# OpenVVC/OpenVVC

Measured on AMD Instinct MI355X. Metric: decoded frames/sec, full rcn back-end decode step (H2D of the recorded picture + MC incl. BDOF/DMVR/affine-PROF/GPM/CIIP + LMCS + inverse transform + ordered intra pass + deblocking + SAO + ALF/CC-ALF + D2H of refined MVs + wait + per-picture digest + publication to the device DPB), 4K 10-bit RA rec, higher is better.
Workload: dtype u16 samples / int16 coefficients / int32 accumulate

## Files before the change

### openvvc_amd/csrc/kernels_alf.hip

```cpp
#include "ovvc_common.hip.h"

#ifndef OV_WPE_ALF
#define OV_WPE_ALF 0
#endif
#if OV_WPE_ALF > 0
#define OV_OCC_ALF __attribute__((amdgpu_waves_per_eu(OV_WPE_ALF)))
#else
#define OV_OCC_ALF
#endif

namespace {

#define TL 32
#define LH 3
#define LW (TL + 2 * LH)
#define LPAD 4
#define LWS 40
#define CH 2
#define CW (TL + 2 * CH)

struct AlfRect { int x0, y0, x1, y1; };
__device__ __forceinline__ AlfRect alf_clamp_rect(int border, int x0, int y0, int s, int w, int h)
{
    AlfRect r = { 0, 0, w - 1, h - 1 };
    if (border & OVHIP_BORDER_LEFT) r.x0 = x0;
    if (border & OVHIP_BORDER_UPPER) r.y0 = y0;
    if (border & OVHIP_BORDER_RIGHT) r.x1 = min(r.x1, x0 + s - 1);
    if (border & OVHIP_BORDER_BOTTOM) r.y1 = min(r.y1, y0 + s - 1);
    return r;
}

__device__ __forceinline__ int alf_clipd(int clip, int ref, int a, int b)
// ... 28 lines not shown
    const int act = min((int)(((sum_h + sum_v) * scale) >> (OV_BD + 4)), 15);
    int c = act == 0 ? 0 : act == 1 ? 1 : act <= 6 ? 2 : act <= 14 ? 3 : 4;
    uint32_t max_hv, min_hv, max_db, min_db, max_dir, min_dir;
    int dir_hv, dir_db, main_dir, sec_dir;
    if (sum_v > sum_h) { max_hv = sum_v; min_hv = sum_h; dir_hv = 1; } else { max_hv = sum_h; min_hv = sum_v; dir_hv = 3; }
    if (sum_d > sum_b) { max_db = sum_d; min_db = sum_b; dir_db = 0; } else { max_db = sum_b; min_db = sum_d; dir_db = 2; }
    if (max_db * min_hv > max_hv * min_db) { max_dir = max_db; min_dir = min_db; main_dir = dir_db; sec_dir = dir_hv; }
    else { max_dir = max_hv; min_dir = min_hv; main_dir = dir_hv; sec_dir = dir_db; }
    if (max_dir * 2 > 9 * min_dir) c += (((main_dir & 1) << 1) + 2) * 5;
    else if (max_dir > 2 * min_dir) c += (((main_dir & 1) << 1) + 1) * 5;
    cls = c;
    const int k = (main_dir << 1) + (sec_dir >> 1);
    tr = (0xDE84 >> (2 * k)) & 3;
}

__device__ __forceinline__ void alf_luma_tile(const ovhip_pic &dst, const ovhip_pic &src, const ovhip_alf_pic &alf, int nb_ctu_w,
                                              int tile0, uint16_t *s_t, uint8_t *s_cls, uint4 *s_sum, int row0, int row1)
{

    const int W = src.w, H = src.h;
    const int tid = threadIdx.x;
    const int ctu = 1 << alf.log2_ctu_s;
    const int ntx = (W + TL - 1) / TL, ntiles = ntx * ((H + TL - 1) / TL);
    for (int tile = tile0; tile < ntiles; tile = ntiles) {
    const int tx0 = (tile % ntx) * TL, ty0 = (tile / ntx) * TL;
    const ovhip_alf_ctu c = alf.ctus[(ty0 >> alf.log2_ctu_s) * nb_ctu_w + (tx0 >> alf.log2_ctu_s)];
    const bool on = c.flags & 4;

    const int b = tid >> 2, r = tid & 3;
    const int bx = (b & 7) * 4, by = (b >> 3) * 4;
    const int ox = tx0 + bx, oy = ty0 + by + r;

    if (!on) {
        if (oy < H && oy >= row0 && oy < row1) {
#pragma unroll
            for (int i = 0; i < 4; ++i) if (ox + i < W) dst.y[oy * dst.stride_y + ox + i] = src.y[oy * src.stride_y + ox + i];
        }
        continue;
    }

    const AlfRect rc = alf_clamp_rect(c.border, tx0 & ~(ctu - 1), ty0 & ~(ctu - 1), ctu, W, H);
    if (tx0 >= rc.x0 + LPAD && tx0 + TL + LPAD <= rc.x1 + 1 && ty0 >= rc.y0 + LH && ty0 + TL + LH <= rc.y1 + 1 && !(src.stride_y & 7)) {
        if (tid < LW * 5) {
            const int yy = tid / 5, q = tid - yy * 5;
            *reinterpret_cast<uint4 *>(s_t + yy * LWS + 8 * q) =
                *reinterpret_cast<const uint4 *>(src.y + (ty0 + yy - LH) * src.stride_y + tx0 - LPAD + 8 * q);
        }
    } else {
        for (int i = tid; i < LW * LWS; i += 256) {
            const int yy = i / LWS, xx = i - yy * LWS;
            const int sy = ov_clip3(ty0 + yy - LH, rc.y0, rc.y1), sx = ov_clip3(tx0 + xx - LPAD, rc.x0, rc.x1);
            s_t[i] = src.y[sy * src.stride_y + sx];
        }
    }
    __syncthreads();

    const int ctu_y0 = ty0 & ~(ctu - 1);
    const bool truncated = ctu_y0 + ctu > H;
    const int vbl = truncated ? H : ctu - 4;
    const int last_local = (ctu_y0 + (truncated ? H - ctu_y0 : ctu) - 1) & (ctu - 1);
    const bool req_vb = (last_local < vbl && last_local >= vbl - 4) || (last_local >= vbl && last_local <= vbl + 3);
    const int vb = ctu_y0 + vbl;

#define T(x, y) ((int)s_t[((y) + LH) * LWS + (x) + LPAD])
    {
        const int cb = tid >> 2, k = tid & 3;
        const int cbx = (cb & 7) * 4, cby = (cb >> 3) * 4;
        const int rr = cby - 2 + 2 * k;
        int above = rr - 1, below = rr + 2;
        if (ty0 + rr + 2 == vb) below = rr + 1;
        if (ty0 + rr == vb)     above = rr;
        uint32_t sv = 0, sh = 0, sd = 0, sb = 0;
        {
            uint32_t ra[6], r0[6], r1[6], rb[6];
            const uint16_t *base = s_t + LH * LWS + cbx;
            auto row3 = [&](int y, uint32_t d6[6]) {
                const uint2 *q2 = reinterpret_cast<const uint2 *>(base + y * LWS);
                const uint2 a = q2[0], b_ = q2[1], c_ = q2[2];
                d6[0] = a.x; d6[1] = a.y; d6[2] = b_.x; d6[3] = b_.y; d6[4] = c_.x; d6[5] = c_.y;
            };
            row3(above, ra); row3(rr, r0); row3(rr + 1, r1); row3(below, rb);
            typedef unsigned short alf_u2 __attribute__((ext_vector_type(2)));
#pragma unroll
            for (int q = 0; q < 4; ++q) {
                const int c0 = 2 * q - 2, c1 = c0 + 1;
                const alf_u2 ctr = __builtin_bit_cast(alf_u2, ALF_PK66(r0, c0, r1, c1));
                const uint32_t y2 = __builtin_bit_cast(uint32_t, ctr + ctr);
#define LAP(acc, A, ca, B, cb, C, cc_, D, cd)                                                                      \
                acc = __builtin_amdgcn_sad_u16(y2, __builtin_bit_cast(uint32_t, __builtin_bit_cast(alf_u2, ALF_PK66(A, ca, B, cb)) + \
                                                                               __builtin_bit_cast(alf_u2, ALF_PK66(C, cc_, D, cd))), acc)
                LAP(sv, ra, c0, r0, c1, r1, c0, rb, c1);
                LAP(sh, r0, c0 + 1, r1, c1 + 1, r0, c0 - 1, r1, c1 - 1);
                LAP(sd, ra, c0 - 1, r0, c1 - 1, r1, c0 + 1, rb, c1 + 1);
                LAP(sb, r1, c0 - 1, rb, c1 - 1, ra, c0 + 1, r0, c1 + 1);
#undef LAP
            }
        }
        const int py = ty0 + cby;
        bool use = true, is_vb = false;
        if (py == vb - 4) { is_vb = true; use = k < 3; }
        if (py == vb)     { is_vb = true; use = k > 0; }
        if (!use) sv = sh = sd = sb = 0;
        (void)is_vb;
        s_sum[tid] = make_uint4(sv, sh, sd, sb);
    }
    __syncthreads();
    if (tid < 64) {
        const uint4 p0 = s_sum[4 * tid], p1 = s_sum[4 * tid + 1], p2 = s_sum[4 * tid + 2], p3 = s_sum[4 * tid + 3];
        const int py = ty0 + (tid >> 3) * 4;
        int cls, tr;
        filter_idx(p0.y + p1.y + p2.y + p3.y, p0.x + p1.x + p2.x + p3.x, p0.z + p1.z + p2.z + p3.z, p0.w + p1.w + p2.w + p3.w,
                   py == vb - 4 || py == vb, cls, tr);
        s_cls[tid] = (uint8_t)(cls | (tr << 5));
    }
    __syncthreads();

    if (oy >= H || oy < row0 || oy >= row1) continue;
    const int ct = s_cls[b];
    const int cls = ct & 31, tr = ct >> 5;
    const int16_t *f = alf.luma_coeff + c.luma_set * OVHIP_ALF_LUMA_SET_SIZE + tr * 25 * 13 + cls * 13;
    const int16_t *cl = alf.luma_clip + c.luma_set * OVHIP_ALF_LUMA_SET_SIZE + tr * 25 * 13 + cls * 13;
    typedef uint32_t alf_u32a2 __attribute__((aligned(2)));
    uint32_t fw[6], cw6[6];
#pragma unroll
    for (int j = 0; j < 6; ++j) { fw[j] = *reinterpret_cast<const alf_u32a2 *>(f + 2 * j); cw6[j] = *reinterpret_cast<const alf_u32a2 *>(cl + 2 * j); }

    int d = 3;
    bool near = false;
    if (req_vb) {
        if (oy < vb && oy >= vb - 4) d = vb - 1 - oy;
        else if (oy >= vb && oy <= vb + 3) d = oy - vb;
        near = (oy == vb - 1) || (oy == vb);
    }
    const int o1 = min(d, 1), o2 = min(d, 2), o3 = min(d, 3);
    const int ly = by + r;
    uint32_t r0[6], p1[6], m1[6], p2[6], m2[6], p3[2], m3[2];
    {
        const uint16_t *base = s_t + LH * LWS + bx;
        auto row3 = [&](int y, uint32_t d6[6]) {
            const uint2 *q = reinterpret_cast<const uint2 *>(base + y * LWS);
            const uint2 a = q[0], b_ = q[1], c_ = q[2];
            d6[0] = a.x; d6[1] = a.y; d6[2] = b_.x; d6[3] = b_.y; d6[4] = c_.x; d6[5] = c_.y;
        };
        auto row1 = [&](int y, uint32_t d2[2]) {
            const uint2 a = reinterpret_cast<const uint2 *>(base + y * LWS)[1];
            d2[0] = a.x; d2[1] = a.y;
        };
        row3(ly, r0); row3(ly + o1, p1); row3(ly - o1, m1); row3(ly + o2, p2); row3(ly - o2, m2);
        row1(ly + o3, p3); row1(ly - o3, m3);
    }
#define S6(d6, c) ((((c) + 4) & 1) ? (int)((d6)[((c) + 4) >> 1] >> 16) : (int)((d6)[((c) + 4) >> 1] & 0xffff))
#define S2(d2, c) (((c) & 1) ? (int)((d2)[(c) >> 1] >> 16) : (int)((d2)[(c) >> 1] & 0xffff))
    alf_s2 cm2 = __builtin_bit_cast(alf_s2, cw6[0]);
    int fsum = 0;
#pragma unroll
    for (int j = 1; j < 6; ++j) cm2 = __builtin_elementwise_min(cm2, __builtin_bit_cast(alf_s2, cw6[j]));
#pragma unroll
    for (int j = 0; j < 6; ++j) fsum = __builtin_amdgcn_sdot2(__builtin_bit_cast(alf_s2, fw[j]), (alf_s2)(1), fsum, false);
    const int cmin = min((int)cm2.x, (int)cm2.y);
    const bool linear = __all(cmin > OV_PIX_MAX);
    uint32_t f2[12], c2[12], nc2[12];
#pragma unroll
    for (int j = 0; j < 6; ++j) {
        f2[2 * j] = __builtin_amdgcn_perm(fw[j], fw[j], 0x01000100u); f2[2 * j + 1] = __builtin_amdgcn_perm(fw[j], fw[j], 0x03020302u);
    }
    if (!linear) {
#pragma unroll
        for (int j = 0; j < 6; ++j) {
            c2[2 * j] = __builtin_amdgcn_perm(cw6[j], cw6[j], 0x01000100u); c2[2 * j + 1] = __builtin_amdgcn_perm(cw6[j], cw6[j], 0x03020302u);
        }
#pragma unroll
        for (int i = 0; i < 12; ++i) nc2[i] = __builtin_bit_cast(uint32_t, (alf_s2)(0) - __builtin_bit_cast(alf_s2, c2[i]));
    }
    int outv[4];
#pragma unroll
    for (int i = 0; i < 4; ++i) {
        const int cur = S6(r0, i);
        const uint32_t n[12] = {
            ALF_PK22(p3, i, m3, i),
            ALF_PK66(p2, i + 1, m2, i - 1), ALF_PK66(p2, i, m2, i), ALF_PK66(p2, i - 1, m2, i + 1),
            ALF_PK66(p1, i + 2, m1, i - 2), ALF_PK66(p1, i + 1, m1, i - 1), ALF_PK66(p1, i, m1, i),
            ALF_PK66(p1, i - 1, m1, i + 1), ALF_PK66(p1, i - 2, m1, i + 2),
            ALF_PK66(r0, i + 3, r0, i - 3), ALF_PK66(r0, i + 2, r0, i - 2), ALF_PK66(r0, i + 1, r0, i - 1) };
        int sum;
        if (linear) {
            sum = -2 * cur * fsum;
#pragma unroll
            for (int k = 0; k < 12; ++k) sum = alf_tap_lin(n[k], f2[k], sum);
        } else {
            const uint32_t cur2 = ALF_PK66(r0, i, r0, i);
            sum = 0;
#pragma unroll
            for (int k = 0; k < 12; ++k) sum = alf_tap(n[k], cur2, c2[k], nc2[k], f2[k], sum);
        }
        sum = near ? (sum + 512) >> 10 : (sum + 64) >> 7;
        outv[i] = ov_clip_bd(sum + cur);
    }
#undef S6
#undef S2
    {
        uint16_t *o = dst.y + oy * dst.stride_y + ox;
        if (ox + 3 < W && !(dst.stride_y & 3)) {
            uint2 v; v.x = (uint32_t)outv[0] | ((uint32_t)outv[1] << 16); v.y = (uint32_t)outv[2] | ((uint32_t)outv[3] << 16);
            *reinterpret_cast<uint2 *>(o) = v;
        } else {
#pragma unroll
            for (int i = 0; i < 4; ++i) if (ox + i < W) o[i] = (uint16_t)outv[i];
        }
    }
    }
#undef T
}

__device__ __forceinline__ void alf_chroma_tile(const ovhip_pic &dst, const ovhip_pic &src, const ovhip_alf_pic &alf, int nb_ctu_w,
                                                int tile0, int comp, uint16_t *s_t, int row0, int row1)
{
    const int W = src.w, H = src.h, Wc = W >> 1, Hc = H >> 1;
    const int tid = threadIdx.x;
    const int ctu = 1 << alf.log2_ctu_s, ctuc = ctu >> 1;
    const int ntx = (Wc + TL - 1) / TL, ntiles = ntx * ((Hc + TL - 1) / TL);
    for (int tile = tile0; tile < ntiles; tile = ntiles) {
    const int tx0 = (tile % ntx) * TL, ty0 = (tile / ntx) * TL;
    const ovhip_alf_ctu c = alf.ctus[((ty0 * 2) >> alf.log2_ctu_s) * nb_ctu_w + ((tx0 * 2) >> alf.log2_ctu_s)];
    const bool on = c.flags & (comp == 1 ? 2 : 1);
    const int cc_idx = comp == 1 ? c.cc_cb_idx : c.cc_cr_idx;
    const uint16_t *sp = comp == 1 ? src.cb : src.cr;
// ... 141 lines not shown
#undef S6
#undef S2
    uint16_t *o = dp + oy * dst.stride_c + tx0 + lx0;
    if (tx0 + lx0 + 3 < Wc && !(dst.stride_c & 3)) {
        uint2 v; v.x = (uint32_t)outv[0] | ((uint32_t)outv[1] << 16); v.y = (uint32_t)outv[2] | ((uint32_t)outv[3] << 16);
        *reinterpret_cast<uint2 *>(o) = v;
    } else {
#pragma unroll
        for (int i = 0; i < 4; ++i) if (tx0 + lx0 + i < Wc) o[i] = (uint16_t)outv[i];
    }
    }
}

__global__ __launch_bounds__(256) OV_OCC_ALF void k_alf(ovhip_pic dst, ovhip_pic src, ovhip_alf_pic alf, int nb_ctu_w, int nl, int nc, int t0_l, int t0_c, int row0, int row1)
{
    __shared__ __attribute__((aligned(16))) uint16_t s_t[(LW > CW ? LW : CW) * LWS];
    __shared__ uint8_t s_cls[64];
    __shared__ __attribute__((aligned(16))) uint4 s_sum[256];
    const int b = blockIdx.x;
    if (b < nl) alf_luma_tile(dst, src, alf, nb_ctu_w, t0_l + (int)ov_xcd_slot_at(b, 0, nl), s_t, s_cls, s_sum, row0, row1);
    else {
        const int comp = 1 + (b - nl) / nc;
        alf_chroma_tile(dst, src, alf, nb_ctu_w, t0_c + (int)ov_xcd_slot_at(b, nl + (comp - 1) * nc, nc), comp, s_t, row0, row1);
    }
}

}

extern "C" int ovhip_alf_launch_rows(ovhip_ctx *ctx, const ovhip_pic *dst, const ovhip_pic *src, const ovhip_alf_pic *alf, int32_t row0, int32_t row1)
{
    if (!ctx || !dst || !src || !alf) return OVHIP_EINVAL;
    OV_DEVICE(ctx);
    if (dst->w != src->w || dst->h != src->h || dst->y == src->y || alf->log2_ctu_s < 6 || alf->log2_ctu_s > 7 ||
        !alf->ctus || !alf->luma_coeff || !alf->luma_clip || !alf->chroma_coeff || !alf->chroma_clip || !alf->cc_coeff)
        return ov_fail(ctx, OVHIP_EINVAL, "ovhip_alf_launch: bad pictures / parameter tables", hipSuccess);
    if (row0 < 0 || row1 > src->h || row0 > row1 || (row0 & 7) || ((row1 & 7) && row1 != src->h))
        return ov_fail(ctx, OVHIP_EINVAL, "ovhip_alf_launch_rows: row window", hipSuccess);
    if (row0 == row1) return OVHIP_OK;
    const int nb_ctu_w = (src->w + (1 << alf->log2_ctu_s) - 1) >> alf->log2_ctu_s;
    const int ntx_l = (src->w + TL - 1) / TL, ntx_c = (src->w / 2 + TL - 1) / TL;
    const int ty0_l = row0 / TL, ty1_l = (row1 + TL - 1) / TL, ty0_c = (row0 / 2) / TL, ty1_c = (row1 / 2 + TL - 1) / TL;
    const int nl = ntx_l * (ty1_l - ty0_l), nc = ntx_c * (ty1_c - ty0_c);
    hipLaunchKernelGGL(k_alf, dim3(nl + 2 * nc), dim3(256), 0, ctx->stream, *dst, *src, *alf, nb_ctu_w, nl, nc, ty0_l * ntx_l, ty0_c * ntx_c, row0, row1);
    OV_LAUNCH_CHECK(ctx, "k_alf");
    return OVHIP_OK;
}

extern "C" int ovhip_alf_launch(ovhip_ctx *ctx, const ovhip_pic *dst, const ovhip_pic *src, const ovhip_alf_pic *alf)
{
    if (!src) return OVHIP_EINVAL;
    return ovhip_alf_launch_rows(ctx, dst, src, alf, 0, src->h);
}
```

### openvvc_amd/csrc/kernels_sao.hip

```cpp
#include "ovvc_common.hip.h"
#include <stdlib.h>

namespace {

#define SAO_TW 64
#define SAO_TH 32

struct Vec8 { int v[8]; };

__device__ __forceinline__ void load8(const uint16_t *p, bool vec, int n, int v[8])
{
    if (vec) {
        const uint4 q = *reinterpret_cast<const uint4 *>(p);
        v[0] = q.x & 0xffff; v[1] = q.x >> 16; v[2] = q.y & 0xffff; v[3] = q.y >> 16;
        v[4] = q.z & 0xffff; v[5] = q.z >> 16; v[6] = q.w & 0xffff; v[7] = q.w >> 16;
    } else {
#pragma unroll
        for (int i = 0; i < 8; ++i) v[i] = i < n ? p[i] : 0;
    }
}

__global__ __launch_bounds__(256) void k_sao(ovhip_pic dst, ovhip_pic src, const ovhip_sao_ctu *__restrict__ prm,
                                              int log2_ctu, int nb_ctu_w, int tiles_y, int tiles_c, int ty0_y, int ty0_c, int row0, int row1)
{
    const int tx = threadIdx.x & 7, ty = threadIdx.x >> 3;
    for (int t = blockIdx.x; t < tiles_y + 2 * tiles_c; t = tiles_y + 2 * tiles_c) {
        const int c = t < tiles_y ? 0 : (t < tiles_y + tiles_c ? 1 : 2);
        const int tt = (int)ov_xcd_slot_at(t, c == 0 ? 0 : (c == 1 ? tiles_y : tiles_y + tiles_c), c == 0 ? tiles_y : tiles_c);
        const int sh = c ? 1 : 0;
        const int w = src.w >> sh, h = src.h >> sh, l2 = log2_ctu - sh;
        const int ntx = (w + SAO_TW - 1) / SAO_TW;
        const int x0 = (tt % ntx) * SAO_TW + tx * 8, y = (tt / ntx + (c ? ty0_c : ty0_y)) * SAO_TH + ty;
        if (x0 >= w || y >= h || y < (row0 >> sh) || y >= (row1 >> sh)) continue;
        int ss, ds;
        const uint16_t *s = ov_plane(src, c, ss) + y * ss;
        uint16_t *d = ov_plane(dst, c, ds) + y * ds;
        const ovhip_sao_ctu *p = &prm[(y >> l2) * nb_ctu_w + (x0 >> l2)];
        const int type = p->type[c];
        const int n = min(8, w - x0);
        const bool vec = n == 8 && !((ss | ds) & 7) && !(((uintptr_t)s | (uintptr_t)d) & 15);
        int v[8], o[8];
        load8(s + x0, vec, n, v);
#pragma unroll
        for (int i = 0; i < 8; ++i) o[i] = v[i];
        if (type == OVHIP_SAO_BAND) {
            const int bp = p->band_position[c];
            const int o0 = p->offset_val[c][0], o1 = p->offset_val[c][1], o2 = p->offset_val[c][2], o3 = p->offset_val[c][3];
#pragma unroll
            for (int i = 0; i < 8; ++i) {
                const int k = ((v[i] >> (OV_BD - 5)) - bp) & 31;
                const int off = k == 0 ? o0 : k == 1 ? o1 : k == 2 ? o2 : k == 3 ? o3 : 0;
                o[i] = ov_clip_bd(v[i] + off);
            }
        } else if (type == OVHIP_SAO_EDGE) {
            const int eo = p->eo_class[c];
            const int dxa = eo == 1 ? 0 : (eo == 3 ? 1 : -1), dya = eo == 0 ? 0 : -1;
            const int bd = p->border, cs = 1 << l2;
            const int cy0 = y & ~(cs - 1), cx0 = x0 & ~(cs - 1);
            const int cx1 = min(cx0 + cs, w) - 1;
            const bool rowskip = eo != 0 && (y == 0 || y == h - 1 || (src.h <= (1 << log2_ctu) && y == (6 >> sh) - 1) ||
                                             ((bd & OVHIP_BORDER_UPPER) && y == cy0) || ((bd & OVHIP_BORDER_BOTTOM) && y == min(cy0 + cs, h) - 1) ||
                                             ((bd & OVHIP_BORDER_ONE_ROW) && y == cy0 + (6 >> sh) - 1));
            const int skip_l = (bd & OVHIP_BORDER_LEFT) ? cx0 : -1, skip_r = (bd & OVHIP_BORDER_RIGHT) ? cx1 : -1;
            if (!rowskip) {
                const int of0 = p->offset_val[c][0], of1 = p->offset_val[c][1], of2 = p->offset_val[c][2],
                          of3 = p->offset_val[c][3], of4 = p->offset_val[c][4];
                int ra[10], rb[10];
                const uint16_t *sa = s + dya * ss, *sb = s - dya * ss;
                load8(sa + x0, vec, n, ra + 1);
                load8(sb + x0, vec, n, rb + 1);
                ra[0] = x0 > 0 ? sa[x0 - 1] : 0; rb[0] = x0 > 0 ? sb[x0 - 1] : 0;
                ra[9] = x0 + 8 < w ? sa[x0 + 8] : 0; rb[9] = x0 + 8 < w ? sb[x0 + 8] : 0;
#pragma unroll
                for (int i = 0; i < 8; ++i) {
                    const int x = x0 + i;
                    if (i < n && !(eo != 1 && (x == 0 || x == w - 1 || x == skip_l || x == skip_r))) {
                        const int a = ra[1 + i + dxa], b = rb[1 + i - dxa];
                        const int idx = 2 + (v[i] > a) - (v[i] < a) + (v[i] > b) - (v[i] < b);
                        const int off = idx == 0 ? of0 : idx == 1 ? of1 : idx == 2 ? of2 : idx == 3 ? of3 : of4;
                        o[i] = ov_clip_bd(v[i] + off);
                    }
                }
            }
        }
        if (vec) {
            uint4 q;
            q.x = o[0] | (o[1] << 16); q.y = o[2] | (o[3] << 16); q.z = o[4] | (o[5] << 16); q.w = o[6] | (o[7] << 16);
            *reinterpret_cast<uint4 *>(d + x0) = q;
        } else {
#pragma unroll
            for (int i = 0; i < 8; ++i) if (i < n) d[x0 + i] = (uint16_t)o[i];
        }
    }
}

}

extern "C" int ovhip_sao_launch_rows(ovhip_ctx *ctx, const ovhip_pic *dst, const ovhip_pic *src,
                                     const ovhip_sao_ctu *d_params, int32_t log2_ctu_s, int32_t row0, int32_t row1)
{
    if (!ctx || !dst || !src || !d_params) return OVHIP_EINVAL;
    OV_DEVICE(ctx);
    if (dst->w != src->w || dst->h != src->h || dst->y == src->y || log2_ctu_s < 5 || log2_ctu_s > 7)
        return ov_fail(ctx, OVHIP_EINVAL, "ovhip_sao_launch: bad pictures / CTU size", hipSuccess);
    if (row0 < 0 || row1 > src->h || row0 > row1 || (row0 & 7) || ((row1 & 7) && row1 != src->h))
        return ov_fail(ctx, OVHIP_EINVAL, "ovhip_sao_launch_rows: row window", hipSuccess);
    if (row0 == row1) return OVHIP_OK;
    const int nb_ctu_w = (src->w + (1 << log2_ctu_s) - 1) >> log2_ctu_s;
// ... 18 lines not shown
```

Measured before the change: 3631.

## Enlarge ALF luma tiles to 4x4 per thread and register-block SAO rows

```diff
diff --git a/openvvc_amd/csrc/kernels_alf.hip b/openvvc_amd/csrc/kernels_alf.hip
--- a/openvvc_amd/csrc/kernels_alf.hip
+++ b/openvvc_amd/csrc/kernels_alf.hip
@@ -12,10 +12,12 @@
 namespace {
 
 #define TL 32
+#define TLL 64
 #define LH 3
-#define LW (TL + 2 * LH)
 #define LPAD 4
 #define LWS 40
+#define LLS 72
+#define LLH (TLL + 2 * LH)
 #define CH 2
 #define CW (TL + 2 * CH)
 
@@ -74,46 +76,105 @@
     tr = (0xDE84 >> (2 * k)) & 3;
 }
 
+__device__ __forceinline__ void alf_lap_pair(const uint32_t ra[6], const uint32_t r0[6], const uint32_t r1[6], const uint32_t rb[6],
+                                             uint32_t &sv, uint32_t &sh, uint32_t &sd, uint32_t &sb)
+{
+    typedef unsigned short alf_u2 __attribute__((ext_vector_type(2)));
+#pragma unroll
+    for (int q = 0; q < 4; ++q) {
+        const int c0 = 2 * q - 2, c1 = c0 + 1;
+        const alf_u2 ctr = __builtin_bit_cast(alf_u2, ALF_PK66(r0, c0, r1, c1));
+        const uint32_t y2 = __builtin_bit_cast(uint32_t, ctr + ctr);
+#define LAP(acc, A, ca, B, cb, C, cc_, D, cd)                                                                      \
+        acc = __builtin_amdgcn_sad_u16(y2, __builtin_bit_cast(uint32_t, __builtin_bit_cast(alf_u2, ALF_PK66(A, ca, B, cb)) + \
+                                                                       __builtin_bit_cast(alf_u2, ALF_PK66(C, cc_, D, cd))), acc)
+        LAP(sv, ra, c0, r0, c1, r1, c0, rb, c1);
+        LAP(sh, r0, c0 + 1, r1, c1 + 1, r0, c0 - 1, r1, c1 - 1);
+        LAP(sd, ra, c0 - 1, r0, c1 - 1, r1, c0 + 1, rb, c1 + 1);
+        LAP(sb, r1, c0 - 1, rb, c1 - 1, ra, c0 + 1, r0, c1 + 1);
+#undef LAP
+    }
+}
+
+struct AlfLumaSet { uint32_t f2[12], c2[12], nc2[12]; int fsum; bool linear; };
+
+__device__ __forceinline__ uint2 alf_luma_row(const uint32_t r0[6], const uint32_t p1[6], const uint32_t m1[6], const uint32_t p2[6],
+                                              const uint32_t m2[6], const uint32_t p3[6], const uint32_t m3[6], bool near, const AlfLumaSet &fs)
+{
+#define S6(d6, c) ((((c) + 4) & 1) ? (int)((d6)[((c) + 4) >> 1] >> 16) : (int)((d6)[((c) + 4) >> 1] & 0xffff))
+    int outv[4];
+#pragma unroll
+    for (int i = 0; i < 4; ++i) {
+        const int cur = S6(r0, i);
+        const uint32_t n[12] = {
+            ALF_PK66(p3, i, m3, i),
+            ALF_PK66(p2, i + 1, m2, i - 1), ALF_PK66(p2, i, m2, i), ALF_PK66(p2, i - 1, m2, i + 1),
+            ALF_PK66(p1, i + 2, m1, i - 2), ALF_PK66(p1, i + 1, m1, i - 1), ALF_PK66(p1, i, m1, i),
+            ALF_PK66(p1, i - 1, m1, i + 1), ALF_PK66(p1, i - 2, m1, i + 2),
+            ALF_PK66(r0, i + 3, r0, i - 3), ALF_PK66(r0, i + 2, r0, i - 2), ALF_PK66(r0, i + 1, r0, i - 1) };
+        int sum;
+        if (fs.linear) {
+            sum = -2 * cur * fs.fsum;
+#pragma unroll
+            for (int k = 0; k < 12; ++k) sum = alf_tap_lin(n[k], fs.f2[k], sum);
+        } else {
+            const uint32_t cur2 = ALF_PK66(r0, i, r0, i);
+            sum = 0;
+#pragma unroll
+            for (int k = 0; k < 12; ++k) sum = alf_tap(n[k], cur2, fs.c2[k], fs.nc2[k], fs.f2[k], sum);
+        }
+        sum = near ? (sum + 512) >> 10 : (sum + 64) >> 7;
+        outv[i] = ov_clip_bd(sum + cur);
+    }
+#undef S6
+    uint2 v; v.x = (uint32_t)outv[0] | ((uint32_t)outv[1] << 16); v.y = (uint32_t)outv[2] | ((uint32_t)outv[3] << 16);
+    return v;
+}
+
 __device__ __forceinline__ void alf_luma_tile(const ovhip_pic &dst, const ovhip_pic &src, const ovhip_alf_pic &alf, int nb_ctu_w,
-                                              int tile0, uint16_t *s_t, uint8_t *s_cls, uint4 *s_sum, int row0, int row1)
+                                              int tile0, uint16_t *s_t, int row0, int row1)
 {
 
     const int W = src.w, H = src.h;
     const int tid = threadIdx.x;
     const int ctu = 1 << alf.log2_ctu_s;
-    const int ntx = (W + TL - 1) / TL, ntiles = ntx * ((H + TL - 1) / TL);
+    const int ntx = (W + TLL - 1) / TLL, ntiles = ntx * ((H + TLL - 1) / TLL);
     for (int tile = tile0; tile < ntiles; tile = ntiles) {
-    const int tx0 = (tile % ntx) * TL, ty0 = (tile / ntx) * TL;
+    const int tx0 = (tile % ntx) * TLL, ty0 = (tile / ntx) * TLL;
     const ovhip_alf_ctu c = alf.ctus[(ty0 >> alf.log2_ctu_s) * nb_ctu_w + (tx0 >> alf.log2_ctu_s)];
     const bool on = c.flags & 4;
 
-    const int b = tid >> 2, r = tid & 3;
-    const int bx = (b & 7) * 4, by = (b >> 3) * 4;
-    const int ox = tx0 + bx, oy = ty0 + by + r;
+    const int bx = (tid & 15) * 4, by = (tid >> 4) * 4;
+    const int ox = tx0 + bx, py = ty0 + by;
+    const bool mine = py < H && py >= row0 && py < row1 && ox < W;
 
     if (!on) {
-        if (oy < H && oy >= row0 && oy < row1) {
-#pragma unroll
-            for (int i = 0; i < 4; ++i) if (ox + i < W) dst.y[oy * dst.stride_y + ox + i] = src.y[oy * src.stride_y + ox + i];
+        if (mine) {
+#pragma unroll
+            for (int r = 0; r < 4; ++r)
+#pragma unroll
+                for (int i = 0; i < 4; ++i)
+                    if (py + r < H && ox + i < W) dst.y[(py + r) * dst.stride_y + ox + i] = src.y[(py + r) * src.stride_y + ox + i];
         }
         continue;
     }
 
     const AlfRect rc = alf_clamp_rect(c.border, tx0 & ~(ctu - 1), ty0 & ~(ctu - 1), ctu, W, H);
-    if (tx0 >= rc.x0 + LPAD && tx0 + TL + LPAD <= rc.x1 + 1 && ty0 >= rc.y0 + LH && ty0 + TL + LH <= rc.y1 + 1 && !(src.stride_y & 7)) {
-        if (tid < LW * 5) {
-            const int yy = tid / 5, q = tid - yy * 5;
-            *reinterpret_cast<uint4 *>(s_t + yy * LWS + 8 * q) =
+    if (tx0 >= rc.x0 + LPAD && tx0 + TLL + LPAD <= rc.x1 + 1 && ty0 >= rc.y0 + LH && ty0 + TLL + LH <= rc.y1 + 1 && !(src.stride_y & 7)) {
+        for (int i = tid; i < LLH * 9; i += 256) {
+            const int yy = i / 9, q = i - yy * 9;
+            *reinterpret_cast<uint4 *>(s_t + yy * LLS + 8 * q) =
                 *reinterpret_cast<const uint4 *>(src.y + (ty0 + yy - LH) * src.stride_y + tx0 - LPAD + 8 * q);
         }
     } else {
-        for (int i = tid; i < LW * LWS; i += 256) {
-            const int yy = i / LWS, xx = i - yy * LWS;
+        for (int i = tid; i < LLH * LLS; i += 256) {
+            const int yy = i / LLS, xx = i - yy * LLS;
             const int sy = ov_clip3(ty0 + yy - LH, rc.y0, rc.y1), sx = ov_clip3(tx0 + xx - LPAD, rc.x0, rc.x1);
             s_t[i] = src.y[sy * src.stride_y + sx];
         }
     }
     __syncthreads();
+    if (!mine) continue;
 
     const int ctu_y0 = ty0 & ~(ctu - 1);
     const bool truncated = ctu_y0 + ctu > H;
@@ -121,155 +182,100 @@
     const int last_local = (ctu_y0 + (truncated ? H - ctu_y0 : ctu) - 1) & (ctu - 1);
     const bool req_vb = (last_local < vbl && last_local >= vbl - 4) || (last_local >= vbl && last_local <= vbl + 3);
     const int vb = ctu_y0 + vbl;
-
-#define T(x, y) ((int)s_t[((y) + LH) * LWS + (x) + LPAD])
-    {
-        const int cb = tid >> 2, k = tid & 3;
-        const int cbx = (cb & 7) * 4, cby = (cb >> 3) * 4;
-        const int rr = cby - 2 + 2 * k;
-        int above = rr - 1, below = rr + 2;
-        if (ty0 + rr + 2 == vb) below = rr + 1;
-        if (ty0 + rr == vb)     above = rr;
-        uint32_t sv = 0, sh = 0, sd = 0, sb = 0;
-        {
+    const bool is_vb = py == vb - 4 || py == vb;
+    const bool at_vb = py + 3 >= vb - 4 && py <= vb + 3;
+
+    const uint16_t *base = s_t + LH * LLS + bx;
+    auto row3 = [&](int y, uint32_t d6[6]) {
+        const uint2 *q2 = reinterpret_cast<const uint2 *>(base + y * LLS);
+        const uint2 a = q2[0], b_ = q2[1], c_ = q2[2];
+        d6[0] = a.x; d6[1] = a.y; d6[2] = b_.x; d6[3] = b_.y; d6[4] = c_.x; d6[5] = c_.y;
+    };
+    uint32_t Rw[10][6];
+#pragma unroll
+    for (int j = 0; j < 10; ++j) row3(by - 3 + j, Rw[j]);
+
+    uint32_t sv = 0, sh = 0, sd = 0, sb = 0;
+    if (!at_vb) {
+#pragma unroll
+        for (int k = 0; k < 4; ++k) alf_lap_pair(Rw[2 * k], Rw[2 * k + 1], Rw[2 * k + 2], Rw[2 * k + 3], sv, sh, sd, sb);
+    } else {
+        for (int k = 0; k < 4; ++k) {
+            if ((py == vb - 4 && k == 3) || (py == vb && k == 0)) continue;
+            const int rr = by - 2 + 2 * k;
+            int above = rr - 1, below = rr + 2;
+            if (ty0 + rr + 2 == vb) below = rr + 1;
+            if (ty0 + rr == vb)     above = rr;
             uint32_t ra[6], r0[6], r1[6], rb[6];
-            const uint16_t *base = s_t + LH * LWS + cbx;
-            auto row3 = [&](int y, uint32_t d6[6]) {
-                const uint2 *q2 = reinterpret_cast<const uint2 *>(base + y * LWS);
-                const uint2 a = q2[0], b_ = q2[1], c_ = q2[2];
-                d6[0] = a.x; d6[1] = a.y; d6[2] = b_.x; d6[3] = b_.y; d6[4] = c_.x; d6[5] = c_.y;
-            };
             row3(above, ra); row3(rr, r0); row3(rr + 1, r1); row3(below, rb);
-            typedef unsigned short alf_u2 __attribute__((ext_vector_type(2)));
-#pragma unroll
-            for (int q = 0; q < 4; ++q) {
-                const int c0 = 2 * q - 2, c1 = c0 + 1;
-                const alf_u2 ctr = __builtin_bit_cast(alf_u2, ALF_PK66(r0, c0, r1, c1));
-                const uint32_t y2 = __builtin_bit_cast(uint32_t, ctr + ctr);
-#define LAP(acc, A, ca, B, cb, C, cc_, D, cd)                                                                      \
-                acc = __builtin_amdgcn_sad_u16(y2, __builtin_bit_cast(uint32_t, __builtin_bit_cast(alf_u2, ALF_PK66(A, ca, B, cb)) + \
-                                                                               __builtin_bit_cast(alf_u2, ALF_PK66(C, cc_, D, cd))), acc)
-                LAP(sv, ra, c0, r0, c1, r1, c0, rb, c1);
-                LAP(sh, r0, c0 + 1, r1, c1 + 1, r0, c0 - 1, r1, c1 - 1);
-                LAP(sd, ra, c0 - 1, r0, c1 - 1, r1, c0 + 1, rb, c1 + 1);
-                LAP(sb, r1, c0 - 1, rb, c1 - 1, ra, c0 + 1, r0, c1 + 1);
-#undef LAP
-            }
-        }
-        const int py = ty0 + cby;
-        bool use = true, is_vb = false;
-        if (py == vb - 4) { is_vb = true; use = k < 3; }
-        if (py == vb)     { is_vb = true; use = k > 0; }
-        if (!use) sv = sh = sd = sb = 0;
-        (void)is_vb;
-        s_sum[tid] = make_uint4(sv, sh, sd, sb);
-    }
-    __syncthreads();
-    if (tid < 64) {
-        const uint4 p0 = s_sum[4 * tid], p1 = s_sum[4 * tid + 1], p2 = s_sum[4 * tid + 2], p3 = s_sum[4 * tid + 3];
-        const int py = ty0 + (tid >> 3) * 4;
-        int cls, tr;
-        filter_idx(p0.y + p1.y + p2.y + p3.y, p0.x + p1.x + p2.x + p3.x, p0.z + p1.z + p2.z + p3.z, p0.w + p1.w + p2.w + p3.w,
-                   py == vb - 4 || py == vb, cls, tr);
-        s_cls[tid] = (uint8_t)(cls | (tr << 5));
-    }
-    __syncthreads();
-
-    if (oy >= H || oy < row0 || oy >= row1) continue;
-    const int ct = s_cls[b];
-    const int cls = ct & 31, tr = ct >> 5;
+            alf_lap_pair(ra, r0, r1, rb, sv, sh, sd, sb);
+        }
+    }
+    int cls, tr;
+    filter_idx(sh, sv, sd, sb, is_vb, cls, tr);
+
     const int16_t *f = alf.luma_coeff + c.luma_set * OVHIP_ALF_LUMA_SET_SIZE + tr * 25 * 13 + cls * 13;
     const int16_t *cl = alf.luma_clip + c.luma_set * OVHIP_ALF_LUMA_SET_SIZE + tr * 25 * 13 + cls * 13;
     typedef uint32_t alf_u32a2 __attribute__((aligned(2)));
     uint32_t fw[6], cw6[6];
 #pragma unroll
     for (int j = 0; j < 6; ++j) { fw[j] = *reinterpret_cast<const alf_u32a2 *>(f + 2 * j); cw6[j] = *reinterpret_cast<const alf_u32a2 *>(cl + 2 * j); }
-
-    int d = 3;
-    bool near = false;
-    if (req_vb) {
-        if (oy < vb && oy >= vb - 4) d = vb - 1 - oy;
-        else if (oy >= vb && oy <= vb + 3) d = oy - vb;
-        near = (oy == vb - 1) || (oy == vb);
-    }
-    const int o1 = min(d, 1), o2 = min(d, 2), o3 = min(d, 3);
-    const int ly = by + r;
-    uint32_t r0[6], p1[6], m1[6], p2[6], m2[6], p3[2], m3[2];
-    {
-        const uint16_t *base = s_t + LH * LWS + bx;
-        auto row3 = [&](int y, uint32_t d6[6]) {
-            const uint2 *q = reinterpret_cast<const uint2 *>(base + y * LWS);
-            const uint2 a = q[0], b_ = q[1], c_ = q[2];
-            d6[0] = a.x; d6[1] = a.y; d6[2] = b_.x; d6[3] = b_.y; d6[4] = c_.x; d6[5] = c_.y;
-        };
-        auto row1 = [&](int y, uint32_t d2[2]) {
-            const uint2 a = reinterpret_cast<const uint2 *>(base + y * LWS)[1];
-            d2[0] = a.x; d2[1] = a.y;
-        };
-        row3(ly, r0); row3(ly + o1, p1); row3(ly - o1, m1); row3(ly + o2, p2); row3(ly - o2, m2);
-        row1(ly + o3, p3); row1(ly - o3, m3);
-    }
-#define S6(d6, c) ((((c) + 4) & 1) ? (int)((d6)[((c) + 4) >> 1] >> 16) : (int)((d6)[((c) + 4) >> 1] & 0xffff))
-#define S2(d2, c) (((c) & 1) ? (int)((d2)[(c) >> 1] >> 16) : (int)((d2)[(c) >> 1] & 0xffff))
+    AlfLumaSet fs;
     alf_s2 cm2 = __builtin_bit_cast(alf_s2, cw6[0]);
-    int fsum = 0;
+    fs.fsum = 0;
 #pragma unroll
     for (int j = 1; j < 6; ++j) cm2 = __builtin_elementwise_min(cm2, __builtin_bit_cast(alf_s2, cw6[j]));
 #pragma unroll
-    for (int j = 0; j < 6; ++j) fsum = __builtin_amdgcn_sdot2(__builtin_bit_cast(alf_s2, fw[j]), (alf_s2)(1), fsum, false);
+    for (int j = 0; j < 6; ++j) fs.fsum = __builtin_amdgcn_sdot2(__builtin_bit_cast(alf_s2, fw[j]), (alf_s2)(1), fs.fsum, false);
     const int cmin = min((int)cm2.x, (int)cm2.y);
-    const bool linear = __all(cmin > OV_PIX_MAX);
-    uint32_t f2[12], c2[12], nc2[12];
+    fs.linear = __all(cmin > OV_PIX_MAX);
 #pragma unroll
     for (int j = 0; j < 6; ++j) {
-        f2[2 * j] = __builtin_amdgcn_perm(fw[j], fw[j], 0x01000100u); f2[2 * j + 1] = __builtin_amdgcn_perm(fw[j], fw[j], 0x03020302u);
-    }
-    if (!linear) {
+        fs.f2[2 * j] = __builtin_amdgcn_perm(fw[j], fw[j], 0x01000100u); fs.f2[2 * j + 1] = __builtin_amdgcn_perm(fw[j], fw[j], 0x03020302u);
+    }
+    if (!fs.linear) {
 #pragma unroll
         for (int j = 0; j < 6; ++j) {
-            c2[2 * j] = __builtin_amdgcn_perm(cw6[j], cw6[j], 0x01000100u); c2[2 * j + 1] = __builtin_amdgcn_perm(cw6[j], cw6[j], 0x03020302u);
-        }
-#pragma unroll
-        for (int i = 0; i < 12; ++i) nc2[i] = __builtin_bit_cast(uint32_t, (alf_s2)(0) - __builtin_bit_cast(alf_s2, c2[i]));
-    }
-    int outv[4];
-#pragma unroll
-    for (int i = 0; i < 4; ++i) {
-        const int cur = S6(r0, i);
-        const uint32_t n[12] = {
-            ALF_PK22(p3, i, m3, i),
-            ALF_PK66(p2, i + 1, m2, i - 1), ALF_PK66(p2, i, m2, i), ALF_PK66(p2, i - 1, m2, i + 1),
-            ALF_PK66(p1, i + 2, m1, i - 2), ALF_PK66(p1, i + 1, m1, i - 1), ALF_PK66(p1, i, m1, i),
-            ALF_PK66(p1, i - 1, m1, i + 1), ALF_PK66(p1, i - 2, m1, i + 2),
-            ALF_PK66(r0, i + 3, r0, i - 3), ALF_PK66(r0, i + 2, r0, i - 2), ALF_PK66(r0, i + 1, r0, i - 1) };
-        int sum;
-        if (linear) {
-            sum = -2 * cur * fsum;
-#pragma unroll
-            for (int k = 0; k < 12; ++k) sum = alf_tap_lin(n[k], f2[k], sum);
-        } else {
-            const uint32_t cur2 = ALF_PK66(r0, i, r0, i);
-            sum = 0;
-#pragma unroll
-            for (int k = 0; k < 12; ++k) sum = alf_tap(n[k], cur2, c2[k], nc2[k], f2[k], sum);
-        }
-        sum = near ? (sum + 512) >> 10 : (sum + 64) >> 7;
-        outv[i] = ov_clip_bd(sum + cur);
-    }
-#undef S6
-#undef S2
-    {
+            fs.c2[2 * j] = __builtin_amdgcn_perm(cw6[j], cw6[j], 0x01000100u); fs.c2[2 * j + 1] = __builtin_amdgcn_perm(cw6[j], cw6[j], 0x03020302u);
+        }
+#pragma unroll
+        for (int i = 0; i < 12; ++i) fs.nc2[i] = __builtin_bit_cast(uint32_t, (alf_s2)(0) - __builtin_bit_cast(alf_s2, fs.c2[i]));
+    }
+
+    uint2 outv[4];
+    if (!(req_vb && at_vb)) {
+#pragma unroll
+        for (int r = 0; r < 4; ++r)
+            outv[r] = alf_luma_row(Rw[r + 3], Rw[r + 4], Rw[r + 2], Rw[r + 5], Rw[r + 1], Rw[r + 6], Rw[r], false, fs);
+    } else {
+        for (int r = 0; r < 4; ++r) {
+            const int oy = py + r;
+            int d = 3;
+            if (oy < vb && oy >= vb - 4) d = vb - 1 - oy;
+            else if (oy >= vb && oy <= vb + 3) d = oy - vb;
+            const bool near = (oy == vb - 1) || (oy == vb);
+            const int o1 = min(d, 1), o2 = min(d, 2), o3 = min(d, 3);
+            const int ly = by + r;
+            uint32_t r0[6], p1[6], m1[6], p2[6], m2[6], p3[6], m3[6];
+            row3(ly, r0); row3(ly + o1, p1); row3(ly - o1, m1); row3(ly + o2, p2); row3(ly - o2, m2); row3(ly + o3, p3); row3(ly - o3, m3);
+            const uint2 v = alf_luma_row(r0, p1, m1, p2, m2, p3, m3, near, fs);
+            if (r == 0) outv[0] = v; else if (r == 1) outv[1] = v; else if (r == 2) outv[2] = v; else outv[3] = v;
+        }
+    }
+#pragma unroll
+    for (int r = 0; r < 4; ++r) {
+        const int oy = py + r;
+        if (oy >= H) continue;
         uint16_t *o = dst.y + oy * dst.stride_y + ox;
         if (ox + 3 < W && !(dst.stride_y & 3)) {
-            uint2 v; v.x = (uint32_t)outv[0] | ((uint32_t)outv[1] << 16); v.y = (uint32_t)outv[2] | ((uint32_t)outv[3] << 16);
-            *reinterpret_cast<uint2 *>(o) = v;
+            *reinterpret_cast<uint2 *>(o) = outv[r];
         } else {
-#pragma unroll
-            for (int i = 0; i < 4; ++i) if (ox + i < W) o[i] = (uint16_t)outv[i];
-        }
-    }
-    }
-#undef T
+            const uint32_t w4[4] = { outv[r].x & 0xffff, outv[r].x >> 16, outv[r].y & 0xffff, outv[r].y >> 16 };
+#pragma unroll
+            for (int i = 0; i < 4; ++i) if (ox + i < W) o[i] = (uint16_t)w4[i];
+        }
+    }
+    }
 }
 
 __device__ __forceinline__ void alf_chroma_tile(const ovhip_pic &dst, const ovhip_pic &src, const ovhip_alf_pic &alf, int nb_ctu_w,
@@ -441,11 +447,9 @@
 
 __global__ __launch_bounds__(256) OV_OCC_ALF void k_alf(ovhip_pic dst, ovhip_pic src, ovhip_alf_pic alf, int nb_ctu_w, int nl, int nc, int t0_l, int t0_c, int row0, int row1)
 {
-    __shared__ __attribute__((aligned(16))) uint16_t s_t[(LW > CW ? LW : CW) * LWS];
-    __shared__ uint8_t s_cls[64];
-    __shared__ __attribute__((aligned(16))) uint4 s_sum[256];
+    __shared__ __attribute__((aligned(16))) uint16_t s_t[LLH * LLS > CW * LWS ? LLH * LLS : CW * LWS];
     const int b = blockIdx.x;
-    if (b < nl) alf_luma_tile(dst, src, alf, nb_ctu_w, t0_l + (int)ov_xcd_slot_at(b, 0, nl), s_t, s_cls, s_sum, row0, row1);
+    if (b < nl) alf_luma_tile(dst, src, alf, nb_ctu_w, t0_l + (int)ov_xcd_slot_at(b, 0, nl), s_t, row0, row1);
     else {
         const int comp = 1 + (b - nl) / nc;
         alf_chroma_tile(dst, src, alf, nb_ctu_w, t0_c + (int)ov_xcd_slot_at(b, nl + (comp - 1) * nc, nc), comp, s_t, row0, row1);
@@ -465,8 +469,8 @@
         return ov_fail(ctx, OVHIP_EINVAL, "ovhip_alf_launch_rows: row window", hipSuccess);
     if (row0 == row1) return OVHIP_OK;
     const int nb_ctu_w = (src->w + (1 << alf->log2_ctu_s) - 1) >> alf->log2_ctu_s;
-    const int ntx_l = (src->w + TL - 1) / TL, ntx_c = (src->w / 2 + TL - 1) / TL;
-    const int ty0_l = row0 / TL, ty1_l = (row1 + TL - 1) / TL, ty0_c = (row0 / 2) / TL, ty1_c = (row1 / 2 + TL - 1) / TL;
+    const int ntx_l = (src->w + TLL - 1) / TLL, ntx_c = (src->w / 2 + TL - 1) / TL;
+    const int ty0_l = row0 / TLL, ty1_l = (row1 + TLL - 1) / TLL, ty0_c = (row0 / 2) / TL, ty1_c = (row1 / 2 + TL - 1) / TL;
     const int nl = ntx_l * (ty1_l - ty0_l), nc = ntx_c * (ty1_c - ty0_c);
     hipLaunchKernelGGL(k_alf, dim3(nl + 2 * nc), dim3(256), 0, ctx->stream, *dst, *src, *alf, nb_ctu_w, nl, nc, ty0_l * ntx_l, ty0_c * ntx_c, row0, row1);
     OV_LAUNCH_CHECK(ctx, "k_alf");
diff --git a/openvvc_amd/csrc/kernels_sao.hip b/openvvc_amd/csrc/kernels_sao.hip
--- a/openvvc_amd/csrc/kernels_sao.hip
+++ b/openvvc_amd/csrc/kernels_sao.hip
@@ -3,95 +3,203 @@
 
 namespace {
 
-#define SAO_TW 64
-#define SAO_TH 32
-
-struct Vec8 { int v[8]; };
-
-__device__ __forceinline__ void load8(const uint16_t *p, bool vec, int n, int v[8])
+#define SAO_TW 128
+#define SAO_TH 64
+#define SAO_WW 64
+#define SAO_WH 32
+
+typedef short sao_s2 __attribute__((ext_vector_type(2)));
+typedef unsigned short sao_u2 __attribute__((ext_vector_type(2)));
+#define SAO_S2(x) __builtin_bit_cast(sao_s2, (uint32_t)(x))
+#define SAO_U2(x) __builtin_bit_cast(sao_u2, (uint32_t)(x))
+#define SAO_U32(x) __builtin_bit_cast(uint32_t, (x))
+
+__device__ __forceinline__ void sao_load_row(const uint16_t *p, bool vec, int n, uint32_t r[4])
 {
     if (vec) {
         const uint4 q = *reinterpret_cast<const uint4 *>(p);
-        v[0] = q.x & 0xffff; v[1] = q.x >> 16; v[2] = q.y & 0xffff; v[3] = q.y >> 16;
-        v[4] = q.z & 0xffff; v[5] = q.z >> 16; v[6] = q.w & 0xffff; v[7] = q.w >> 16;
+        r[0] = q.x; r[1] = q.y; r[2] = q.z; r[3] = q.w;
     } else {
 #pragma unroll
-        for (int i = 0; i < 8; ++i) v[i] = i < n ? p[i] : 0;
-    }
-}
-
-__global__ __launch_bounds__(256) void k_sao(ovhip_pic dst, ovhip_pic src, const ovhip_sao_ctu *__restrict__ prm,
-                                              int log2_ctu, int nb_ctu_w, int tiles_y, int tiles_c, int ty0_y, int ty0_c, int row0, int row1)
-{
-    const int tx = threadIdx.x & 7, ty = threadIdx.x >> 3;
-    for (int t = blockIdx.x; t < tiles_y + 2 * tiles_c; t = tiles_y + 2 * tiles_c) {
-        const int c = t < tiles_y ? 0 : (t < tiles_y + tiles_c ? 1 : 2);
-        const int tt = (int)ov_xcd_slot_at(t, c == 0 ? 0 : (c == 1 ? tiles_y : tiles_y + tiles_c), c == 0 ? tiles_y : tiles_c);
-        const int sh = c ? 1 : 0;
-        const int w = src.w >> sh, h = src.h >> sh, l2 = log2_ctu - sh;
-        const int ntx = (w + SAO_TW - 1) / SAO_TW;
-        const int x0 = (tt % ntx) * SAO_TW + tx * 8, y = (tt / ntx + (c ? ty0_c : ty0_y)) * SAO_TH + ty;
-        if (x0 >= w || y >= h || y < (row0 >> sh) || y >= (row1 >> sh)) continue;
-        int ss, ds;
-        const uint16_t *s = ov_plane(src, c, ss) + y * ss;
-        uint16_t *d = ov_plane(dst, c, ds) + y * ds;
-        const ovhip_sao_ctu *p = &prm[(y >> l2) * nb_ctu_w + (x0 >> l2)];
-        const int type = p->type[c];
-        const int n = min(8, w - x0);
-        const bool vec = n == 8 && !((ss | ds) & 7) && !(((uintptr_t)s | (uintptr_t)d) & 15);
-        int v[8], o[8];
-        load8(s + x0, vec, n, v);
-#pragma unroll
-        for (int i = 0; i < 8; ++i) o[i] = v[i];
-        if (type == OVHIP_SAO_BAND) {
-            const int bp = p->band_position[c];
-            const int o0 = p->offset_val[c][0], o1 = p->offset_val[c][1], o2 = p->offset_val[c][2], o3 = p->offset_val[c][3];
-#pragma unroll
-            for (int i = 0; i < 8; ++i) {
-                const int k = ((v[i] >> (OV_BD - 5)) - bp) & 31;
-                const int off = k == 0 ? o0 : k == 1 ? o1 : k == 2 ? o2 : k == 3 ? o3 : 0;
-                o[i] = ov_clip_bd(v[i] + off);
+        for (int j = 0; j < 4; ++j)
+            r[j] = (2 * j < n ? (uint32_t)p[2 * j] : 0u) | (2 * j + 1 < n ? (uint32_t)p[2 * j + 1] << 16 : 0u);
+    }
+}
+
+__device__ __forceinline__ uint32_t sao_from_left(uint32_t v) { return (uint32_t)__builtin_amdgcn_update_dpp(0, (int)v, 0x111, 0xf, 0xf, true); }
+__device__ __forceinline__ uint32_t sao_from_right(uint32_t v) { return (uint32_t)__builtin_amdgcn_update_dpp(0, (int)v, 0x101, 0xf, 0xf, true); }
+
+__device__ __forceinline__ void sao_at_left(const uint32_t c[4], uint32_t lw, uint32_t o[4])
+{
+    o[0] = __builtin_amdgcn_alignbit(c[0], lw, 16);
+#pragma unroll
+    for (int j = 1; j < 4; ++j) o[j] = __builtin_amdgcn_alignbit(c[j], c[j - 1], 16);
+}
+__device__ __forceinline__ void sao_at_right(const uint32_t c[4], uint32_t rw, uint32_t o[4])
+{
+#pragma unroll
+    for (int j = 0; j < 3; ++j) o[j] = __builtin_amdgcn_alignbit(c[j + 1], c[j], 16);
+    o[3] = __builtin_amdgcn_alignbit(rw, c[3], 16);
+}
+
+__device__ __forceinline__ uint32_t sao_add(uint32_t c, uint32_t sel, uint32_t t0, uint32_t t1)
+{
+    const sao_u2 s = SAO_U2(c) + SAO_U2(__builtin_amdgcn_perm(t1, t0, sel));
+    return SAO_U32(__builtin_elementwise_min(__builtin_elementwise_sub_sat(s, (sao_u2)(128)), (sao_u2)(OV_PIX_MAX)));
+}
+__device__ __forceinline__ sao_s2 sao_sign2(sao_s2 d)
+{
+    uint32_t r;
+    asm("v_pk_max_i16 %0, %1, %2\n\tv_pk_min_i16 %0, %0, %3" : "=&v"(r) : "v"(SAO_U32(d)), "v"(0xffffffffu), "v"(0x00010001u));
+    return SAO_S2(r);
+}
+__device__ __forceinline__ uint32_t sao_edge2(uint32_t c, uint32_t a, uint32_t b, uint32_t t0, uint32_t t1)
+{
+    const sao_s2 sa = sao_sign2(SAO_S2(c) - SAO_S2(a)), sb = sao_sign2(SAO_S2(c) - SAO_S2(b));
+    return sao_add(c, SAO_U32(sa + sb + (sao_s2)(0x0c02)), t0, t1);
+}
+__device__ __forceinline__ uint32_t sao_band2(uint32_t c, uint32_t bp2, uint32_t t0, uint32_t t1)
+{
+    const sao_u2 k = ((SAO_U2(c) >> (sao_u2)(OV_BD - 5)) - SAO_U2(bp2)) & (sao_u2)(31);
+    return sao_add(c, SAO_U32(__builtin_elementwise_min(k, (sao_u2)(4))) | 0x0c000c00u, t0, t1);
+}
+
+template <bool U>
+__device__ __forceinline__ void sao_group(const ovhip_pic &dst, const ovhip_pic &src, const ovhip_sao_ctu *__restrict__ prm, int log2_ctu,
+                                          int nb_ctu_w, int c, int wx0, int wy0, int row0, int row1)
+{
+    const int lane = threadIdx.x & 63, tx = lane & 7;
+    const int sh = c ? 1 : 0;
+    const int w = src.w >> sh, h = src.h >> sh, l2 = log2_ctu - sh;
+    const int x0 = wx0 + tx * 8, y0 = wy0 + (lane >> 3) * 4;
+    const int yhi = min(h, row1 >> sh);
+    const bool live = x0 < w && y0 >= (row0 >> sh) && y0 < yhi;
+    int ss, ds;
+    const uint16_t *sp = ov_plane(src, c, ss);
+    uint16_t *dp = ov_plane(dst, c, ds);
+    const uint16_t *s = sp + y0 * ss + x0;
+    uint16_t *d = dp + y0 * ds + x0;
+
+    int pi = U || !live ? (wy0 >> l2) * nb_ctu_w + (wx0 >> l2) : (y0 >> l2) * nb_ctu_w + (x0 >> l2);
+    if (U) pi = __builtin_amdgcn_readfirstlane(pi);
+    const uint32_t *q = reinterpret_cast<const uint32_t *>(prm + pi);
+    const uint32_t q0 = q[0], q1 = q[1], q2 = q[2];
+    const int type = (int)((((uint64_t)q1 << 32 | q0) >> (8 * c)) & 0xff);
+    const int bp = (int)((((uint64_t)q1 << 32 | q0) >> (24 + 8 * c)) & 0xff);
+    const int eo = (int)((((uint64_t)q2 << 32 | q1) >> (16 + 8 * c)) & 0xff);
+    const int bd = (q2 >> 8) & 0xff;
+    const uint32_t *qo = q + (c == 0 ? 3 : (c == 1 ? 5 : 8));
+    const uint32_t e0 = qo[0], e1 = qo[1], e2 = qo[2];
+    const uint64_t four = c == 1 ? ((uint64_t)e1 << 32 | e0) >> 16 | (uint64_t)(e2 & 0xffff) << 48 : ((uint64_t)e1 << 32 | e0);
+    const uint32_t of4 = c == 1 ? e2 >> 16 : e2 & 0xffff;
+    const uint32_t t0 = ((uint32_t)(four & 0xff) | (uint32_t)((four >> 8) & 0xff00) | (uint32_t)((four >> 16) & 0xff0000) |
+                         (uint32_t)((four >> 24) & 0xff000000)) ^ 0x80808080u;
+    const uint32_t t1 = type == OVHIP_SAO_BAND ? 0x80u : (of4 & 0xff) ^ 0x80u;
+
+    const int n = live ? min(8, w - x0) : 0;
+    const bool vec = n == 8 && !((ss | ds) & 7) && !(((uintptr_t)sp | (uintptr_t)dp) & 15);
+    const bool edge = type == OVHIP_SAO_EDGE;
+    const bool outer = !U || (edge && eo != 0);
+    const bool sides = !U || (edge && eo != 1);
+
+    uint32_t R[6][4];
+    bool have[6];
+#pragma unroll
+    for (int k = 0; k < 6; ++k) {
+        const int y = y0 - 1 + k;
+        have[k] = live && y >= 0 && y < h && (k == 0 || k == 5 ? outer : true);
+        R[k][0] = R[k][1] = R[k][2] = R[k][3] = 0;
+        if (have[k]) sao_load_row(s + (k - 1) * ss, vec, n, R[k]);
+    }
+    uint32_t L[6], Rt[6];
+#pragma unroll
+    for (int k = 0; k < 6; ++k) { L[k] = sao_from_left(R[k][3]); Rt[k] = sao_from_right(R[k][0]); }
+    if (sides && tx == 0) {
+#pragma unroll
+        for (int k = 0; k < 6; ++k) L[k] = have[k] && x0 > 0 ? (uint32_t)s[(k - 1) * ss - 1] << 16 : 0u;
+    }
+    if (sides && tx == 7) {
+#pragma unroll
+        for (int k = 0; k < 6; ++k) Rt[k] = have[k] && x0 + 8 < w ? (uint32_t)s[(k - 1) * ss + 8] : 0u;
+    }
+
+    uint32_t O[4][4];
+#pragma unroll
+    for (int r = 0; r < 4; ++r)
+#pragma unroll
+        for (int j = 0; j < 4; ++j) O[r][j] = R[r + 1][j];
+    if (type == OVHIP_SAO_BAND) {
+        const uint32_t bp2 = (uint32_t)bp * 0x00010001u;
+#pragma unroll
+        for (int r = 0; r < 4; ++r)
+#pragma unroll
+            for (int j = 0; j < 4; ++j) O[r][j] = sao_band2(R[r + 1][j], bp2, t0, t1);
+    } else if (edge) {
+#pragma unroll
+        for (int r = 0; r < 4; ++r) {
+            uint32_t a[4], b[4];
+            if (eo == 0) { sao_at_left(R[r + 1], L[r + 1], a); sao_at_right(R[r + 1], Rt[r + 1], b); }
+            else if (eo == 1) {
+#pragma unroll
+                for (int j = 0; j < 4; ++j) { a[j] = R[r][j]; b[j] = R[r + 2][j]; }
             }
-        } else if (type == OVHIP_SAO_EDGE) {
-            const int eo = p->eo_class[c];
-            const int dxa = eo == 1 ? 0 : (eo == 3 ? 1 : -1), dya = eo == 0 ? 0 : -1;
-            const int bd = p->border, cs = 1 << l2;
-            const int cy0 = y & ~(cs - 1), cx0 = x0 & ~(cs - 1);
+            else if (eo == 3) { sao_at_right(R[r], Rt[r], a); sao_at_left(R[r + 2], L[r + 2], b); }
+            else { sao_at_left(R[r], L[r], a); sao_at_right(R[r + 2], Rt[r + 2], b); }
+#pragma unroll
+            for (int j = 0; j < 4; ++j) O[r][j] = sao_edge2(R[r + 1][j], a[j], b[j], t0, t1);
+        }
+        const bool one_row = src.h <= (1 << log2_ctu);
+        if (x0 == 0 || x0 + 8 >= w || y0 == 0 || y0 + 4 >= h || bd != 0 || (one_row && y0 < 8)) {
+            const int cs = 1 << l2;
+            const int cy0 = y0 & ~(cs - 1), cx0 = x0 & ~(cs - 1);
             const int cx1 = min(cx0 + cs, w) - 1;
-            const bool rowskip = eo != 0 && (y == 0 || y == h - 1 || (src.h <= (1 << log2_ctu) && y == (6 >> sh) - 1) ||
-                                             ((bd & OVHIP_BORDER_UPPER) && y == cy0) || ((bd & OVHIP_BORDER_BOTTOM) && y == min(cy0 + cs, h) - 1) ||
-                                             ((bd & OVHIP_BORDER_ONE_ROW) && y == cy0 + (6 >> sh) - 1));
             const int skip_l = (bd & OVHIP_BORDER_LEFT) ? cx0 : -1, skip_r = (bd & OVHIP_BORDER_RIGHT) ? cx1 : -1;
-            if (!rowskip) {
-                const int of0 = p->offset_val[c][0], of1 = p->offset_val[c][1], of2 = p->offset_val[c][2],
-                          of3 = p->offset_val[c][3], of4 = p->offset_val[c][4];
-                int ra[10], rb[10];
-                const uint16_t *sa = s + dya * ss, *sb = s - dya * ss;
-                load8(sa + x0, vec, n, ra + 1);
-                load8(sb + x0, vec, n, rb + 1);
-                ra[0] = x0 > 0 ? sa[x0 - 1] : 0; rb[0] = x0 > 0 ? sb[x0 - 1] : 0;
-                ra[9] = x0 + 8 < w ? sa[x0 + 8] : 0; rb[9] = x0 + 8 < w ? sb[x0 + 8] : 0;
-#pragma unroll
-                for (int i = 0; i < 8; ++i) {
-                    const int x = x0 + i;
-                    if (i < n && !(eo != 1 && (x == 0 || x == w - 1 || x == skip_l || x == skip_r))) {
-                        const int a = ra[1 + i + dxa], b = rb[1 + i - dxa];
-                        const int idx = 2 + (v[i] > a) - (v[i] < a) + (v[i] > b) - (v[i] < b);
-                        const int off = idx == 0 ? of0 : idx == 1 ? of1 : idx == 2 ? of2 : idx == 3 ? of3 : of4;
-                        o[i] = ov_clip_bd(v[i] + off);
-                    }
+            uint32_t cm[4];
+#pragma unroll
+            for (int j = 0; j < 4; ++j) {
+                const int xa = x0 + 2 * j, xb = xa + 1;
+                cm[j] = eo == 1 ? 0u : ((xa == 0 || xa == w - 1 || xa == skip_l || xa == skip_r ? 0xffffu : 0u) |
+                                        (xb == 0 || xb == w - 1 || xb == skip_l || xb == skip_r ? 0xffff0000u : 0u));
+            }
+#pragma unroll
+            for (int r = 0; r < 4; ++r) {
+                const int y = y0 + r;
+                const bool rowskip = eo != 0 && (y == 0 || y == h - 1 || (one_row && y == (6 >> sh) - 1) ||
+                                                 ((bd & OVHIP_BORDER_UPPER) && y == cy0) || ((bd & OVHIP_BORDER_BOTTOM) && y == min(cy0 + cs, h) - 1) ||
+                                                 ((bd & OVHIP_BORDER_ONE_ROW) && y == cy0 + (6 >> sh) - 1));
+#pragma unroll
+                for (int j = 0; j < 4; ++j) {
+                    const uint32_t m = rowskip ? 0xffffffffu : cm[j];
+                    O[r][j] = (O[r][j] & ~m) | (R[r + 1][j] & m);
                 }
             }
         }
+    }
+#pragma unroll
+    for (int r = 0; r < 4; ++r) {
+        if (!live || y0 + r >= yhi) continue;
         if (vec) {
-            uint4 q;
-            q.x = o[0] | (o[1] << 16); q.y = o[2] | (o[3] << 16); q.z = o[4] | (o[5] << 16); q.w = o[6] | (o[7] << 16);
-            *reinterpret_cast<uint4 *>(d + x0) = q;
+            *reinterpret_cast<uint4 *>(d + r * ds) = make_uint4(O[r][0], O[r][1], O[r][2], O[r][3]);
         } else {
 #pragma unroll
-            for (int i = 0; i < 8; ++i) if (i < n) d[x0 + i] = (uint16_t)o[i];
+            for (int i = 0; i < 8; ++i) if (i < n) d[r * ds + i] = (uint16_t)(O[r][i >> 1] >> (16 * (i & 1)));
         }
     }
+}
+
+__global__ __launch_bounds__(256) void k_sao(ovhip_pic dst, ovhip_pic src, const ovhip_sao_ctu *__restrict__ prm,
+                                              int log2_ctu, int nb_ctu_w, int tiles_y, int tiles_c, int ty0_y, int ty0_c, int row0, int row1)
+{
+    const int t = blockIdx.x, wv = threadIdx.x >> 6;
+    const int c = t < tiles_y ? 0 : (t < tiles_y + tiles_c ? 1 : 2);
+    const int tt = (int)ov_xcd_slot_at(t, c == 0 ? 0 : (c == 1 ? tiles_y : tiles_y + tiles_c), c == 0 ? tiles_y : tiles_c);
+    const int sh = c ? 1 : 0;
+    const int w = src.w >> sh, h = src.h >> sh;
+    const int ntx = (w + SAO_TW - 1) / SAO_TW;
+    const int wx0 = (tt % ntx) * SAO_TW + (wv & 1) * SAO_WW, wy0 = (tt / ntx + (c ? ty0_c : ty0_y)) * SAO_TH + (wv >> 1) * SAO_WH;
+    if (wx0 >= w || wy0 >= h || wy0 + SAO_WH <= (row0 >> sh) || wy0 >= (row1 >> sh)) return;
+    if (log2_ctu - sh >= 6 && !((uintptr_t)prm & 3)) sao_group<true>(dst, src, prm, log2_ctu, nb_ctu_w, c, wx0, wy0, row0, row1);
+    else sao_group<false>(dst, src, prm, log2_ctu, nb_ctu_w, c, wx0, wy0, row0, row1);
 }
 
 }
```

Result: no change. 3669, median of 2 (+1.0%).
